# CRIMAC-WP4-Machine-learning/CRIMAC-classifiers-unet

Hardware: AMD Instinct MI355X
Metric: echogram patches/sec (4ch 256x256), training step (fwd+weighted CE+bwd+SGD) (higher is better)
Workload: dtype bf16; 1 GPU; BASELINE configs[1]: U-Net (depth 5, 64 filters) train step, batch 32 x 4x256x256 per GPU; global_batch=32, precision=bf16, start_filts=64, parallelism=dp1, ranks=1, launcher=single process

## Files before the change

### crimac_classifiers_unet_amd/csrc/elementwise.hip

```cpp
#include <stdarg.h>
#include <stdlib.h>

#include <mutex>

#include "common.h"

static thread_local char g_err[512] = "";
void crimac_set_error(const char* fmt, ...) {
  va_list ap;
  va_start(ap, fmt);
  vsnprintf(g_err, sizeof(g_err), fmt, ap);
  va_end(ap);
}
extern "C" const char* crimac_last_error(void) { return g_err; }
extern "C" int crimac_version(void) { return CRIMAC_ABI_VERSION; }
extern "C" int crimac_layer_desc_size(void) { return (int)sizeof(crimac_layer_desc); }

namespace {

#ifdef CRIMAC_STREAM_FORWARD
#define CRIMAC_ROW(x, M) (x)
#else
#define CRIMAC_ROW(x, M) ((M) - 1 - (x))
#endif
// ... 606 lines not shown
      for (int j = 0; j < 8; ++j) {
        int best = 0;
        float bv = av[0][j];
#pragma unroll
        for (int d = 1; d < 4; ++d)
          if (av[d][j] > bv) { bv = av[d][j]; best = d; }
        arg[j] = best;
      }
#pragma unroll
      for (int d = 0; d < 4; ++d) {
        float o[8];
        if (ds) load8s(ds + pix[d] * ds_ld + c0, o);
#pragma unroll
        for (int j = 0; j < 8; ++j) {
          o[j] = (ds ? o[j] : 0.f) + (arg[j] == d ? g[j] : 0.f);
          if constexpr (BNB) o[j] = storage_round<T>(o[j]);
        }
        if (da) store8(da + pix[d] * da_ld + c0, o);
        if constexpr (BNB) bnb_accum_v(k, yv[d], o, d1, d2);
      }
    }
  }
  if constexpr (BNB) bnb_flush(bnb, lds, C, c0, d1, d2, 256);
}

__device__ __forceinline__ float bn_bwd_dy(float yv, float g, float sc, float sh, float mu, float is, float k1, float k2) {
#pragma clang fp contract(off)
  const float act = __builtin_fmaf(yv, sc, sh);
  const float dz = act > 0.f ? g : 0.f;
  const float xh = (yv - mu) * is;
  return sc * __builtin_fmaf(-xh, k2, dz - k1);
}

template <typename T>
__global__ __launch_bounds__(256) void bn_bwd_reduce_kernel(const T* __restrict__ da, long da_ld,
                                                            const T* __restrict__ y, long y_ld,
                                                            const float* __restrict__ scale,
                                                            const float* __restrict__ shift,
                                                            const float* __restrict__ mean,
                                                            const float* __restrict__ invstd, long M,
                                                            int C, double* sum_dz, double* sum_dzx) {
  const int c0t = (threadIdx.x % (C / 8)) * 8;
  float sc[8], sh[8], mu[8], is[8];
#pragma unroll
  for (int j = 0; j < 8; ++j) {
    sc[j] = scale[c0t + j]; sh[j] = shift[c0t + j]; mu[j] = mean[c0t + j]; is[j] = invstd[c0t + j];
  }
  colreduce<T, double, 2>(M, C,
                          [&](long m, int c0, float (&q0)[8], float (&q1)[8]) {
                            float g[8], yv[8];
                            load8(da + m * da_ld + c0, g);
                            load8(y + m * y_ld + c0, yv);
#pragma unroll
                            for (int j = 0; j < 8; ++j) {
                              const float act = yv[j] * sc[j] + sh[j];
                              const float dz = act > 0.f ? g[j] : 0.f;
                              q0[j] = dz;
                              q1[j] = dz * (yv[j] - mu[j]) * is[j];
                            }
                          },
                          sum_dz, sum_dzx);
}

template <typename T, typename TD = T>
__global__ __launch_bounds__(256) void bn_bwd_apply_kernel(
    const T* __restrict__ da, long da_ld, const T* __restrict__ y, long y_ld,
// ... 141 lines not shown
    load8s(dp + r * dp_ld + c0, g);
    long pix[4];
#pragma unroll
    for (int d = 0; d < 4; ++d) {
      pix[d] = (b * H + 2 * yp + (d >> 1)) * (long)W + 2 * xp + (d & 1);
      load8s(y + pix[d] * y_ld + c0, yv[d]);
#pragma unroll
      for (int j = 0; j < 8; ++j) av[d][j] = storage_round<TA>(fmaxf(yv[d][j] * sc[j] + sh[j], 0.f));
    }
    int arg[8];
#pragma unroll
    for (int j = 0; j < 8; ++j) {
      int best = 0;
      float bv = av[0][j];
#pragma unroll
      for (int d = 1; d < 4; ++d)
        if (av[d][j] > bv) { bv = av[d][j]; best = d; }
      arg[j] = best;
    }
#pragma unroll
    for (int d = 0; d < 4; ++d) {
      float o[8];
      if (ds) load8s(ds + pix[d] * ds_ld + c0, o);
#pragma unroll
      for (int j = 0; j < 8; ++j) {
        const float dav = storage_round<T>((ds ? o[j] : 0.f) + (arg[j] == d ? g[j] : 0.f));
        o[j] = bn_bwd_dy(yv[d][j], dav, sc[j], sh[j], mu[j], is[j], k1[j], k2[j]);
      }
      store8(dy + pix[d] * dy_ld + c0, o);
    }
  }
}

template <typename T, int NC, typename TR = T>
__global__ __launch_bounds__(256) void head_fwd_kernel(const T* __restrict__ x, long x_ld, int Cin,
                                                       const float* __restrict__ w,
                                                       const float* __restrict__ bias,
                                                       float* __restrict__ logits, long npix, long HW,
                                                       int softmax, const float* __restrict__ bn_scale,
                                                       const float* __restrict__ bn_shift) {
  const int lp = Cin / 8;
  const int sub = threadIdx.x % lp;
  float bsc[8], bsh[8];
#pragma unroll
  for (int j = 0; j < 8; ++j) {
    bsc[j] = bn_scale ? bn_scale[sub * 8 + j] : 1.f;
    bsh[j] = bn_scale ? bn_shift[sub * 8 + j] : 0.f;
  }
  float wr[NC][8];
#pragma unroll
  for (int o = 0; o < NC; ++o)
#pragma unroll
    for (int j = 0; j < 8; ++j) wr[o][j] = w[o * Cin + sub * 8 + j];
  const long ppb = 256 / lp;
  for (long p0 = (long)blockIdx.x * ppb; p0 < npix; p0 += (long)gridDim.x * ppb) {
    const long p = p0 + threadIdx.x / lp;
    float acc[NC];
#pragma unroll
    for (int o = 0; o < NC; ++o) acc[o] = 0.f;
    if (p < npix) {
      float v[8];
      load8(x + p * x_ld + sub * 8, v);
      if (bn_scale) {
#pragma unroll
        for (int j = 0; j < 8; ++j) v[j] = storage_round<TR>(fmaxf(v[j] * bsc[j] + bsh[j], 0.f));
      }
// ... 150 lines not shown
  long pb[UNR], phw[UNR];
#pragma unroll
  for (int u = 0; u < UNR; ++u) { pb[u] = (p + u * step) / HW; phw[u] = (p + u * step) % HW; }
  for (; p < npix; p += UNR * step) {
    float g[UNR][NC], v[UNR][8], yv[UNR][8];
    bool ok[UNR];
#pragma unroll
    for (int u = 0; u < UNR; ++u) {
      const long pu = p + u * step;
      ok[u] = pu < npix;
      if (phw[u] >= HW) { phw[u] -= HW; pb[u] += 1; }
      if (ok[u]) {
#pragma unroll
        for (int o = 0; o < NC; ++o) g[u][o] = dl[(pb[u] * NC + o) * HW + phw[u]];
        if (x) load8s(x + pu * x_ld + sub * 8, v[u]);
        if constexpr (BNB) load8s(reinterpret_cast<const T*>(bnb.y) + pu * bnb.y_ld + sub * 8, yv[u]);
      }
      pb[u] += step_b;
      phw[u] += step_hw;
    }
#pragma unroll
    for (int u = 0; u < UNR; ++u) {
      if (!ok[u]) continue;
      const long pu = p + u * step;
      float o8[8];
      if constexpr (BNB) {
        if (!x) {
#pragma unroll
          for (int j = 0; j < 8; ++j) v[u][j] = storage_round<TX>(fmaxf(yv[u][j] * k.sc[j] + k.sh[j], 0.f));
        }
      }
#pragma unroll
      for (int j = 0; j < 8; ++j) {
        float s = 0.f;
#pragma unroll
        for (int o = 0; o < NC; ++o) { s += g[u][o] * wr[o][j]; gw[o][j] += g[u][o] * v[u][j]; }
        o8[j] = s;
      }
      if (sub == 0)
#pragma unroll
        for (int o = 0; o < NC; ++o) gb[o] += g[u][o];
      if constexpr (BNB) {
#pragma unroll
        for (int j = 0; j < 8; ++j) o8[j] = storage_round<T>(o8[j]);
      }
      store8(dx + pu * dx_ld + sub * 8, o8);
      if constexpr (BNB) bnb_accum_v(k, yv[u], o8, d1, d2);
    }
  }
#pragma unroll
  for (int o = 0; o < NC; ++o) {
#pragma unroll
    for (int j = 0; j < 8; ++j) atomicAdd(&lds[o * Cin + sub * 8 + j], gw[o][j]);
    if (sub == 0) atomicAdd(&lds[NC * Cin + o], gb[o]);
  }
  __syncthreads();
  for (int i = threadIdx.x; i < NC * Cin; i += 256) atomicAdd(&dw[i], lds[i]);
  if (threadIdx.x < NC) atomicAdd(&db[threadIdx.x], lds[NC * Cin + threadIdx.x]);
  if constexpr (BNB) bnb_flush(bnb, lds_bnb, Cin, sub * 8, d1, d2, 256);
}

__device__ __forceinline__ long load_label(const void* labels, int nbytes, long i) {
  if (nbytes == 8) return ((const long long*)labels)[i];
  if (nbytes == 4) return ((const int*)labels)[i];
  return ((const short*)labels)[i];
}

template <int NC>
__global__ __launch_bounds__(256) void wce_fwd_kernel(const float* __restrict__ logits,
                                                      const void* __restrict__ labels, int lbytes,
                                                      const float* __restrict__ cw, int ignore,
                                                      long npix, long HW, double* sums) {
  __shared__ double red[2][4];
  double s0 = 0.0, s1 = 0.0;
  auto pixel = [&](long y, const float (&z)[NC]) {
    if (y == ignore) return;
    float mx = -INFINITY;
#pragma unroll
    for (int o = 0; o < NC; ++o) mx = fmaxf(mx, z[o]);
// ... 531 lines not shown
    return head_fwd_launch<hp_t, hp_t>(x, x_ld, Cin, w, b, logits, B * HW, HW, ncls, softmax, bn_scale, bn_shift, ST);
  }
  CRIMAC_FOR_STORAGE(prec, T, return head_fwd_launch<T>(x, x_ld, Cin, w, b, logits, B * HW, HW, ncls, softmax, bn_scale,
                                                        bn_shift, ST));
}

template <typename T, typename TX = T>
static int head_bwd_launch(const float* dl, const void* x, long x_ld, int Cin, const float* w, void* dx,
                           long dx_ld, float* dw, float* db, long npix, long HW, int ncls, const BnbArgs& bnb,
                           hipStream_t st) {
  const int lp = Cin / 8;
  int grid = grid_for(npix, (256 / lp) * 32);
  if (grid > 1024) grid = 1024;
  const size_t lds = (size_t)(ncls * Cin + ncls + (bnb.sum_dz ? 2 * Cin : 0)) * sizeof(float);
#define HB(NC, BNB)                                                                                          \
  hipLaunchKernelGGL((head_bwd_kernel<T, NC, BNB, TX>), dim3(whole_rounds(head_bwd_kernel<T, NC, BNB, TX>, lds, grid)), dim3(256), lds, st, dl, (const TX*)x, x_ld,   \
                     Cin, w, (T*)dx, dx_ld, dw, db, npix, HW, bnb)
  if (bnb.sum_dz) {
    if (ncls == 2) HB(2, true); else if (ncls == 3) HB(3, true); else HB(4, true);
  } else {
    if (ncls == 2) HB(2, false); else if (ncls == 3) HB(3, false); else HB(4, false);
  }
#undef HB
  CRIMAC_LAUNCH_CHECK();
  return CRIMAC_OK;
}

extern "C" int crimac_head_bwd(int prec, const float* dlogits, const void* x, long x_ld, int Cin,
                               const float* w, void* dx, long dx_ld, float* dw, float* db, int B, int H,
                               int W, int ncls, const void* bnb_y, long bnb_y_ld, const float* bnb_vec,
                               long bnb_stride, double* stat_sum, double* stat_sumsq, int stat_replicas,
                               void* stream) {
  PREC_OK("head_bwd");
  CRIMAC_REQUIRE(dlogits && w && dx && dw && db && B > 0 && H > 0 && W > 0, "head_bwd: bad arguments");
  CRIMAC_REQUIRE(x || (bnb_y && stat_sum), "head_bwd: x may only be NULL together with the fused BatchNorm sums");
  CRIMAC_REQUIRE(ncls >= 2 && ncls <= 4, "head_bwd: ncls=%d unsupported (2..4)", ncls);
  CRIMAC_REQUIRE(head_cin_ok(Cin) && (!x || (x_ld >= Cin && x_ld % 8 == 0)) && dx_ld >= Cin && dx_ld % 8 == 0,
                 "head_bwd: Cin=%d must be 8*2^k <= 512", Cin);
  CRIMAC_REQUIRE(bnb_args_ok(bnb_y, bnb_y_ld, bnb_vec, bnb_stride, stat_sum, stat_sumsq, stat_replicas, Cin),
                 "head_bwd: bad arguments of the fused BatchNorm-backward sums");
  const long HW = (long)H * W;
  const BnbArgs bnb{bnb_y, bnb_y_ld, bnb_vec, bnb_stride, stat_sum, stat_sumsq, stat_replicas};
  CRIMAC_FOR_STORAGE2(prec, T, TX, return (head_bwd_launch<T, TX>(dlogits, x, x_ld, Cin, w, dx, dx_ld, dw, db, B * HW, HW, ncls,
                                                                    bnb, ST)));
}

extern "C" int crimac_wce_fwd(const float* logits, const void* labels, int label_bytes,
                              const float* class_w, int ncls, int ignore_index, int B, int H, int W,
                              double* sums, void* stream) {
  CRIMAC_REQUIRE(logits && labels && class_w && sums && B > 0 && H > 0 && W > 0, "wce_fwd: bad arguments");
  CRIMAC_REQUIRE(label_bytes == 2 || label_bytes == 4 || label_bytes == 8, "wce_fwd: label_bytes=%d", label_bytes);
  CRIMAC_REQUIRE(ncls >= 2 && ncls <= 4, "wce_fwd: ncls=%d unsupported (2..4)", ncls);
  const long HW = (long)H * W, npix = B * HW;
  int grid = grid_for(npix, 256 * 8);
  if (grid > 512) grid = 512;
#define WF(NC)                                                                                     \
  hipLaunchKernelGGL(wce_fwd_kernel<NC>, dim3(grid), dim3(256), 0, ST, logits, labels, label_bytes, \
                     class_w, ignore_index, npix, HW, sums)
  if (ncls == 2) WF(2); else if (ncls == 3) WF(3); else WF(4);
#undef WF
  CRIMAC_LAUNCH_CHECK();
  return CRIMAC_OK;
}

extern "C" int crimac_wce_bwd(const float* logits, const void* labels, int label_bytes,
                              const float* class_w, int ncls, int ignore_index, int B, int H, int W,
                              const double* sums, float upstream, float* dlogits, void* stream) {
  CRIMAC_REQUIRE(logits && labels && class_w && sums && dlogits && B > 0 && H > 0 && W > 0,
                 "wce_bwd: bad arguments");
  CRIMAC_REQUIRE(label_bytes == 2 || label_bytes == 4 || label_bytes == 8, "wce_bwd: label_bytes=%d", label_bytes);
  CRIMAC_REQUIRE(ncls >= 2 && ncls <= 4, "wce_bwd: ncls=%d unsupported (2..4)", ncls);
  const long HW = (long)H * W, npix = B * HW;
  const int grid = grid_for(npix, 256 * 4);
#define WB(NC)                                                                                     \
  hipLaunchKernelGGL(wce_bwd_kernel<NC>, dim3(whole_rounds(wce_bwd_kernel<NC>, 0, grid)), dim3(256), 0, ST, logits, labels, label_bytes, \
                     class_w, ignore_index, npix, HW, sums, upstream, dlogits)
  if (ncls == 2) WB(2); else if (ncls == 3) WB(3); else WB(4);
// ... 51 lines not shown
```

### crimac_classifiers_unet_amd/engine.py

```python
from __future__ import annotations

import ctypes as C
import os

import torch

from . import hip
from .hip import Act, call, ptr


def _on_device(fn):
    import functools

    @functools.wraps(fn)
    def wrapped(self, *a, **kw):
        if getattr(self, "device", None) is None:
            self.bind()
        dev = self.device
        if dev is None or dev.type != "cuda":
            return fn(self, *a, **kw)
        with torch.cuda.device(dev):
            return fn(self, *a, **kw)
    return wrapped

# ... 605 lines not shown
        if t is None or tuple(t.shape) != tuple(shape) or t.dtype != dtype:
            t = torch.empty(shape, dtype=dtype, device=self.device)
            self._bufs[key] = t
        return t

    def _wfrag_geometry(self, B, H, W):
        es = 4 if self.is_hp else 2
        small = (B * H * W - 1) * (2 * self.sf) * es + 2 * self.sf * es < (1 << 31)
        if small == getattr(self, "_wfrag_on", True):
            return
        self._wfrag_on = small
        for pks in (self.pk_main, self.pk_eval, self.pk16):
            for key, pk in pks.items():
                ok = pk.get("frag_ok") or (self.pk_main.get(key, {}).get("frag_ok", (False, False)) if pks is self.pk_eval else None)
                if ok is None:
                    continue
                if "fwd_frag" in pk:
                    pk["fwd_frag"] = bool(small and ok[0])
                if "dg_frag" in pk:
                    pk["dg_frag"] = bool(small and ok[1])
        self._ltab = self._ltab16 = None
        self._packed_groups = set()
        self._train_pack_dirty = self._eval_pack_dirty = True

    def _geom(self, B, H, W):
        self._wfrag_geometry(B, H, W)
        D = self.depth
        if H % (2 ** (D - 1)) or W % (2 ** (D - 1)):
            raise ValueError(f"H, W must be divisible by {2 ** (D - 1)} (got {H}x{W})")
        return [(H >> i, W >> i, B * (H >> i) * (W >> i)) for i in range(D)]

    fuse_bn_bwd = True
    fuse_unpool_apply = None
    fuse_head_bn = True

    def _conv3x3(self, x: Act, pk, bias, out: Act, B, H, W, cin, cout, relu, dgrad=False, cin_real=None,
                 stats=None, bnb=None, cols=None, out_planes=False, stat_reps=None):
        flops = 2.0 * 9 * (cin_real or cin) * cout * B * H * W
        relu = (hip.EPI_RELU if relu else 0) | (hip.EPI_OUT_PLANES if (out_planes and self.is_hp) else 0)
        if pk.get("narrow"):
            return self._conv3x3_narrow(x, pk, bias, out, B, H, W, cin, cout, relu, dgrad, stats, cols, stat_reps, flops)
        if self.is_hp and cin_real is not None and cin_real <= 4 and cin == CIN_PAD and not dgrad:
            relu |= hip.EPI_CIN4
        w_hi, w_lo = ptr(pk["dg_hi" if dgrad else "fwd_hi"]), ptr(pk["dg_lo" if dgrad else "fwd_lo"])
        if pk.get("dg_frag" if dgrad else "fwd_frag"):
            relu |= hip.EPI_WFRAG
        prec = self.prec_bwd if dgrad else self.prec
        mode, s0, s1, by, by_ld, bvec = 0, None, None, None, 0, None
        reps = stat_reps or self._nrep(cout)
        if stats is not None:
            mode, s0, s1 = 1, ptr(stats[0]), ptr(stats[1])
        elif bnb is not None and self.fuse_bn_bwd:
            blk, y = bnb
            mode, s0, s1 = 2, ptr(self._stat(blk, 0)), ptr(self._stat(blk, 1))
            by, by_ld, bvec = y.p, y.ld, ptr(self._bnf(blk, 0))
        if cols is not None:
            call("crimac_conv3x3_cols", prec, x.p, x.ld, B, H, W, cin, cout, w_hi, w_lo, ptr(bias),
                 out.p, out.ld, relu, mode, s0, s1, reps, by, by_ld, bvec, self.cmax,
                 cols[0], cols[1], flops=flops * cols[1] / cout, mfmas=hip.MFMAS_PER_PRODUCT[prec])
            return mode != 0
        call("crimac_conv3x3", prec, x.p, x.ld, B, H, W, cin, cout, w_hi, w_lo, ptr(bias),
             out.p, out.ld, relu, mode, s0, s1, reps, by, by_ld, bvec, self.cmax,
             flops=flops, mfmas=hip.MFMAS_PER_PRODUCT[prec])
        return mode != 0

    def _conv3x3_narrow(self, x: Act, pk, bias, out: Act, B, H, W, cin, cout, flags, dgrad, stats, cols, stat_reps, flops):
# ... 317 lines not shown
                    self._bn_act(b2, y2, a2, None, B, h, w, M)
                saved[f"d{j}"] = (cur, catA, y1, a1, y2, a2)
            else:
                pe1, pe2 = self.pk_eval[b1.conv_key], self.pk_eval[b2.conv_key]
                self._conv3x3(catA, pe1, pe1["bias"], a1, B, h, w, 2 * c, c, relu=True, out_planes=True)
                self._conv3x3(a1, pe2, pe2["bias"], a2, B, h, w, c, c, relu=True, out_planes=True)
            cur = a2
        logits = out if out is not None else torch.empty((B, self.n_classes, H, W), dtype=torch.float32,
                                                         device=self.device)
        if self.lmi:
            if meta is None:
                raise ValueError("UNet_LateMetInject needs the metadata tensor")
            w64, wm = self._lmi_weights()
            call("crimac_head_fwd", self.prec, cur.p, cur.ld, self.sf, ptr(w64), ptr(self.P["conv_final.bias"]),
                 ptr(logits), B, H, W, self.n_classes, 0,
                 ptr(self._bnf(head_bn, 2)) if head_bn is not None else None,
                 ptr(self._bnf(head_bn, 3)) if head_bn is not None else None)
            m = self._buf("lmi.m", (B * H * W,), torch.float32)
            call("crimac_meta_mlp_fwd", ptr(meta), self.meta_channels, B, H, W, *self._mlp(), ptr(m))
            call("crimac_meta_inject_fwd", ptr(m), ptr(wm), ptr(logits), B, H, W, self.n_classes, 1 if softmax else 0)
            saved["meta"] = meta
        else:
            call("crimac_head_fwd", self.prec, cur.p, cur.ld, self.sf, ptr(self.P["conv_final.weight"]),
                 ptr(self.P["conv_final.bias"]), ptr(logits), B, H, W, self.n_classes, 1 if softmax else 0,
                 ptr(self._bnf(head_bn, 2)) if head_bn is not None else None,
                 ptr(self._bnf(head_bn, 3)) if head_bn is not None else None)
        saved["head_in"] = cur if head_bn is None else None
        self.saved = saved if training else None
        if training:
            self.forward_generation += 1
        return logits

    def _block_bwd(self, tag, b, da: Act, y: Act, x_in: Act, B, h, w, M, dx_out: Act, reduce_done=False,
                   next_bn=None, bias_from_stats=None, unpool_src=None):
        world = self._sync_world()
        folded = reduce_done and self.fold_bn_finalize and world == 1
        if folded:
            pass
        elif reduce_done:
            call("crimac_sum_replicas", ptr(self._stat(b, 0)), self._nrep(b.cout), b.cout, b.cout,
                 ptr(self._stat(b, 2)), None, ptr(self._stat(b, 1)), ptr(self._stat(b, 3)))
        else:
            call("crimac_bn_bwd_reduce", self.prec, da.p, da.ld, y.p, y.ld, ptr(self._bnf(b, 2)),
                 ptr(self._bnf(b, 3)), ptr(self._bnf(b, 0)), ptr(self._bnf(b, 1)), M, b.cout,
                 ptr(self._stat(b, 2)), ptr(self._stat(b, 3)))
        dy = Act(self._buf(f"{tag}.dy", (M, b.cout), torch.float16 if self.bwd16 else None), b.cout)
        prec_apply = self.prec_bwd if self.bwd16 else self.prec
        dgamma, dbeta = self.G[b.bn_key + ".weight"], self.G[b.bn_key + ".bias"]
        if world > 1:
            import torch.distributed as dist
            dgamma.copy_(self._stat(b, 3))
            dbeta.copy_(self._stat(b, 2))
            dist.all_reduce(self._stat_pair(b), group=UNetEngine._bn_group)
            scr = self._buf("g.syncbn.scratch", (2, self.cmax), torch.float32)
            dgamma, dbeta = scr[0], scr[1]
        if unpool_src is not None:
            if not folded:
                raise RuntimeError("unpool_src needs the folded BatchNorm-backward path")
            dp_, ds_ = unpool_src
            call("crimac_unpool_bn_bwd_apply_replicas", prec_apply, dp_.p, dp_.ld, ds_.p if ds_ is not None else None,
                 ds_.ld if ds_ is not None else 0, y.p, y.ld, ptr(self._bnf(b, 0)), self.cmax, ptr(self._stat(b, 0)),
                 ptr(self._stat(b, 1)), self._nrep(b.cout), M, dy.p, dy.ld, B, h, w, b.cout, ptr(dgamma), ptr(dbeta))
        elif folded:
            call("crimac_bn_bwd_apply_replicas", prec_apply, da.p, da.ld, y.p, y.ld, ptr(self._bnf(b, 0)), self.cmax,
                 ptr(self._stat(b, 0)), ptr(self._stat(b, 1)), self._nrep(b.cout), M, M, b.cout, dy.p, dy.ld,
                 ptr(dgamma), ptr(dbeta))
        else:
            call("crimac_bn_bwd_apply", prec_apply, da.p, da.ld, y.p, y.ld, ptr(self._bnf(b, 2)),
                 ptr(self._bnf(b, 3)), ptr(self._bnf(b, 0)), ptr(self._bnf(b, 1)), ptr(self._stat(b, 2)),
                 ptr(self._stat(b, 3)), M, M * world, b.cout, dy.p, dy.ld, ptr(dgamma), ptr(dbeta), None)
        self._wgrad(self.prec_bwd, 0, dy.p, dy.ld, b.cout, x_in.p, x_in.ld, b.cin_pad, B, h, w, b.conv_key,
                    flops=2.0 * 9 * b.cin * b.cout * B * h * w)
        fused = False
        if dx_out is not None:
            stats = None
            if bias_from_stats is not None:
                per = 2 * STAT_REPLICAS * 2 * self.cmax
                lvl = bias_from_stats[2]
                scr = self.bias_scr[lvl * per:(lvl + 1) * per]
                stats = (scr[:per // 2], scr[per // 2:])
            C_up = bias_from_stats[1] if bias_from_stats is not None else 0
            side = self._side[0] if (self._side is not None and len(self._side) == 1) else None
            side_ok = side is not None and not self._gloo_ranks()
            if b.narrow and bias_from_stats is not None:
                self._conv3x3(dy, self.pk[b.conv_key], None, dx_out, B, h, w, b.cout, b.cin, relu=False, dgrad=True,
                              stats=stats, cols=(0, C_up), out_planes=True)
                if side_ok:
                    ev = self._side_events[self._side_i % len(self._side_events)]
                    self._side_i += 1
                    ev.record()
                    with torch.cuda.stream(side):
                        side.wait_event(ev)
                        self._conv3x3(dy, self.pk[b.conv_key], None, dx_out, B, h, w, b.cout, b.cin, relu=False,
                                      dgrad=True, cols=(C_up, C_up))
                        done = torch.cuda.Event()
# ... 85 lines not shown
        if [g for g, _ in bounds] != sorted(starts) or bounds[-1][1] != 0 or not bounds[0][1] < lo_dec:
            raise RuntimeError("unexpected parameter order in the flat buffer")
        for k, (o, _, _) in self.layout.items():
            if (o >= lo_dec) != (k.startswith(dec) or k.startswith("conv_final") or k.startswith("post_processing_weights")):
                raise RuntimeError(f"unexpected parameter order in the flat buffer at {k}")
        ranges, hi = [(lo_dec, self.n_flat)], lo_dec
        for _, lo in bounds:
            ranges.append((lo, hi))
            hi = lo
        return ranges

    @_on_device
    def backward(self, dlogits, on_ready=None, before_join=None):
        ranges = self.grad_ranges() if on_ready is not None else None
        s = self.saved
        if s is None:
            raise RuntimeError("backward() needs a preceding train-mode forward()")
        B, H, W = s["B"], s["H"], s["W"]
        geo = self._geom(B, H, W)
        D = self.depth
        self._skip_done = {}
        self._unpacked = {}
        self._wg_pending, self._wg_launches = [], 0
        self._dup16 = {}
        self._plan_dw(B, H, W)
        self.flat_g.zero_()
        if not self.use_wgrad_partials:
            self.dw_packed.zero_()
        self.stat[2:].zero_()
        self.bias_scr.zero_()
        dlogits = dlogits.contiguous().float()
        head_in = s["head_in"]
        h, w, M = geo[0]
        d_cur = Act(self._buf("g.head", (M, self.sf)), self.sf)
        head_fused = self.fuse_bn_bwd and D >= 2
        if head_in is None and not head_fused:
            raise RuntimeError("head input was not materialised (fuse_head_bn) but the fused BatchNorm sums are off")
        w_head, g_head = ptr(self.P["conv_final.weight"]), self.G["conv_final.weight"]
        if self.lmi:
            w64, wm = self._lmi_weights()
            g64 = self._buf("lmi.g64", (self.n_classes, self.sf), torch.float32)
            gwm = self._buf("lmi.gwm", (self.n_classes,), torch.float32)
            g64.zero_()
            gwm.zero_()
            pre = "post_processing_weights.main."
            call("crimac_meta_bwd", ptr(dlogits), ptr(s["meta"]), self.meta_channels, B, H, W, self.n_classes, ptr(wm),
                 *self._mlp(), ptr(gwm), *[ptr(self.G[pre + k]) for k in
                                          ("0.weight", "0.bias", "2.weight", "2.bias", "4.weight", "4.bias")])
            w_head, g_head = ptr(w64), g64
        call("crimac_head_bwd", self.prec, ptr(dlogits), head_in.p if head_in is not None else None,
             head_in.ld if head_in is not None else 0, self.sf,
             w_head, d_cur.p, d_cur.ld, ptr(g_head),
             ptr(self.G["conv_final.bias"]), B, H, W, self.n_classes,
             *self._bnb_args(self.dec[D - 2][1], s[f"d{D - 2}"][4] if head_fused else None))
        if self.lmi:
            gw = self.G["conv_final.weight"].view(self.n_classes, self.sf + 1)
            gw[:, :self.sf].copy_(g64)
            gw[:, self.sf].copy_(gwm)
        skip_grad = {}
        cur_done = head_fused
        for j in reversed(range(D - 1)):
            L = D - 2 - j
            h, w, M = geo[L]
            c = self.sf * 2 ** L
            u = self.ups[j]
            b1, b2 = self.dec[j]
            x_prev, catA, y1, a1, y2, a2 = s[f"d{j}"]
            da1 = Act(self._buf(f"g.d{j}.a1", (M, c)), c)
            fused = self._block_bwd(f"g.d{j}.2", b2, d_cur, y2, a1, B, h, w, M, da1, next_bn=(b1, y1),
                                    reduce_done=cur_done)
            dcat = Act(self._buf(f"g.d{j}.cat", (M, 2 * c)), 2 * c)
            self._block_bwd(f"g.d{j}.1", b1, da1, y1, catA, B, h, w, M, dcat, reduce_done=fused,
                            bias_from_stats=(self.G[u.key + ".bias"], c, j))
            dup = self._dup16.get(j) or dcat.slice(0, c)
            skip_grad[L] = dcat.slice(c, c)
            hp, wp, Mp = geo[L + 1]
            if u.up1x1:
                dup = self._up1x1_adjoint(dup, u, B, hp, wp)
                self._wgrad1x1(dup, x_prev, u, Mp)
            else:
                self._wgrad(self.prec_bwd, 1, x_prev.p, x_prev.ld, u.cin, dup.p, dup.ld, u.cout, B, hp, wp, u.key,
                            flops=2.0 * 4 * u.cin * u.cout * B * hp * wp)
            d_prev = Act(self._buf(f"g.d{j}.xprev", (Mp, u.cin)), u.cin)
            nxt = (self.dec[j - 1][1], s[f"d{j - 1}"][4]) if j > 0 else (self.enc[D - 1][1], s[f"e{D - 1}"][3])
            cur_done = self._upconv_dgrad(dup, u, d_prev, B, hp, wp, next_bn=nxt)
            d_cur = d_prev
        self._unpack_group(0, on_ready, ranges[0] if ranges else None)
        d_pool = None
        for i in reversed(range(D)):
            h, w, M = geo[i]
            c = self.sf * 2 ** i
            b1, b2 = self.enc[i]
            x_in, y1, a1, y2, a2 = s[f"e{i}"]
            unpool_src = None
            if i == D - 1:
                da2 = d_cur
            else:
                ds = skip_grad[i]
                ev = self._skip_done.pop(D - 2 - i, None)
                if ev is not None:
                    torch.cuda.current_stream().wait_event(ev)
                if (self.fuse_unpool_apply and self.fuse_bn_bwd and self.fold_bn_finalize
                        and self._sync_world() == 1):
# ... 256 lines not shown
```

### crimac_classifiers_unet_amd/hip.py

```python
from __future__ import annotations

import ctypes as C
import os

import torch

from . import build as _build

PREC_BF16 = 0
PREC_F32X3 = 1
PREC_F32X6 = 2
PREC_FP16 = 3
PREC_F32H3 = 4
PREC_H3P = 5
PREC_H3F_BWD = 6
PREC_NAMES = {"bf16": PREC_BF16, "f32x3": PREC_F32X3, "f32x6": PREC_F32X6, "fp16": PREC_FP16, "f32h3": PREC_F32H3,
              "h3p": PREC_H3P, "h3f": PREC_H3P}
MFMAS_PER_PRODUCT = {PREC_BF16: 1, PREC_FP16: 1, PREC_F32X3: 3, PREC_F32H3: 3, PREC_H3P: 3, PREC_F32X6: 6, PREC_H3F_BWD: 1}
PREC_PLANES = {PREC_BF16: 1, PREC_F32X3: 2, PREC_F32X6: 3, PREC_FP16: 1, PREC_F32H3: 2, PREC_H3P: 2}
PLANES_FP16 = 1 | 16 | 32
PLANES_F32H3 = 2 | 16 | (8 << 8)
PLANES_FWD_FRAG = 65536
PLANES_INTERLEAVED = 64
PLANES_H3P = 2 | 16 | 32 | PLANES_INTERLEAVED | 128 | (8 << 8)
PREC_PLANES_ARG = {PREC_BF16: 1, PREC_F32X3: 2, PREC_F32X6: 3, PREC_FP16: PLANES_FP16, PREC_F32H3: PLANES_F32H3,
                   PREC_H3P: PLANES_H3P}
EPI_RELU, EPI_OUT_PLANES, EPI_CIN4 = 1, 2, 4
EPI_WFRAG = 16
EPI_WROWS = 32
NARROW_DGRAD = 64
LAYER_FWD_FRAG, LAYER_DG_FRAG = 16, 32
LAYER_CONV3X3, LAYER_UPCONV2X2, LAYER_CONV1X1 = 0, 1, 2
PREC_BACKWARD = {PREC_F32H3: PREC_F32X3}
PREC_16BIT = (PREC_BF16, PREC_FP16)

ABI_VERSION = 10

_vp, _i, _l, _f = C.c_void_p, C.c_int, C.c_long, C.c_float

SIGNATURES = {
    "crimac_igemm_conv": [_i, _vp, _l, _i, _i, _i, _i, _i, _i, _i, _i, _i, _i, _i, _vp, _vp, _vp, _i,
                          _vp, _l, _i, _i, _i, _vp],
    "crimac_conv3x3": [_i, _vp, _l, _i, _i, _i, _i, _i, _vp, _vp, _vp, _vp, _l, _i, _i, _vp, _vp, _i,
                       _vp, _l, _vp, _l, _vp],
    "crimac_conv3x3_pool": [_i, _vp, _l, _i, _i, _i, _i, _i, _vp, _vp, _vp, _vp, _l, _i, _vp, _l, _vp],
    "crimac_conv3x3_cols": [_i, _vp, _l, _i, _i, _i, _i, _i, _vp, _vp, _vp, _vp, _l, _i, _i, _vp, _vp, _i,
                            _vp, _l, _vp, _l, _i, _i, _vp],
    "crimac_upconv2x2_dgrad_bnb": [_vp, _l, _i, _i, _i, _i, _i, _vp, _vp, _l, _vp, _l, _vp, _l, _vp, _vp, _i, _vp],
    "crimac_upconv2x2_dgrad_bnb_prec": [_i, _vp, _l, _i, _i, _i, _i, _i, _vp, _vp, _l, _vp, _l, _vp, _l, _vp, _vp, _i,
                                        _vp],
    "crimac_sum_replicas": [_vp, _i, _l, _i, _vp, _vp, _vp, _vp, _vp],
    "crimac_wgrad": [_i, _i, _vp, _l, _i, _vp, _l, _i, _i, _i, _i, _vp, _i, _vp],
    "crimac_wgrad_partials": [_i, _i, _vp, _l, _i, _vp, _l, _i, _i, _i, _i, _vp, _l, _i, _vp],
    "crimac_wgrad_group": [_i, _vp, _i, _i, _vp, _i, _vp, _vp, _vp],
    "crimac_conv1x1_up2x": [_i, _vp, _l, _i, _i, _i, _i, _i, _vp, _vp, _vp, _vp, _vp, _l, _vp],
    "crimac_up2x_adjoint": [_i, _vp, _l, _i, _i, _i, _i, _vp, _l, _vp],
    "crimac_conv1x1_dgrad": [_i, _vp, _l, _i, _i, _i, _i, _i, _vp, _vp, _vp, _l, _vp],
    "crimac_conv1x1_wgrad": [_i, _vp, _l, _i, _vp, _l, _i, _l, _vp, _vp],
    "crimac_conv3x3_narrow": [_i, _vp, _l, _i, _i, _i, _i, _i, _vp, _i, _i, _i, _vp, _vp, _vp, _l, _vp, _vp, _i, _i,
                              _vp],
    "crimac_upconv2x2_narrow": [_i, _vp, _l, _i, _i, _i, _i, _i, _vp, _vp, _vp, _l, _i, _vp],
    "crimac_upconv2x2_dgrad_narrow": [_i, _vp, _l, _i, _i, _i, _i, _i, _vp, _vp, _l, _vp],
    "crimac_pack_conv3x3": [_vp, _i, _i, _i, _vp, _i, _vp, _vp, _vp, _vp, _vp],
    "crimac_pack_upconv2x2": [_vp, _i, _i, _i, _vp, _vp, _vp, _vp, _vp],
    "crimac_unpack_wgrad_conv3x3": [_vp, _i, _i, _i, _vp, _vp],
    "crimac_unpack_wgrad_upconv2x2": [_vp, _i, _i, _vp, _vp],
    "crimac_pack_layers": [_vp, _i, _i, _vp],
    "crimac_unpack_wgrad_layers": [_vp, _i, _vp],
    "crimac_nchw_to_nhwc": [_i, _vp, _vp, _i, _i, _i, _i, _l, _vp],
    "crimac_colstats": [_i, _vp, _l, _l, _i, _vp, _vp, _vp],
    "crimac_colsum_f32": [_i, _vp, _l, _l, _i, _vp, _vp],
    "crimac_bn_finalize": [_vp, _vp, _i, _l, _i, _vp, _vp, _f, _f, _vp, _vp, _vp, _vp, _vp, _vp, _vp, _vp],
    "crimac_bn_act_pool": [_i, _vp, _l, _vp, _vp, _i, _vp, _l, _vp, _l, _i, _i, _i, _i, _vp],
    "crimac_bn_train_act_pool": [_i, _vp, _l, _vp, _vp, _i, _l, _vp, _vp, _f, _f, _vp, _vp, _vp, _vp, _l, _i, _vp, _l,
                                 _vp, _l, _i, _i, _i, _i, _vp],
    "crimac_unpool_add": [_i, _vp, _l, _vp, _l, _vp, _l, _vp, _l, _i, _i, _i, _i, _vp, _l, _vp, _l, _vp, _vp, _i,
                          _vp],
    "crimac_bn_bwd_reduce": [_i, _vp, _l, _vp, _l, _vp, _vp, _vp, _vp, _l, _i, _vp, _vp, _vp],
    "crimac_bn_bwd_apply": [_i, _vp, _l, _vp, _l, _vp, _vp, _vp, _vp, _vp, _vp, _l, _l, _i, _vp, _l, _vp,
                            _vp, _vp, _vp],
    "crimac_bn_bwd_apply_replicas": [_i, _vp, _l, _vp, _l, _vp, _l, _vp, _vp, _i, _l, _l, _i, _vp, _l, _vp, _vp, _vp],
    "crimac_unpool_bn_bwd_apply_replicas": [_i, _vp, _l, _vp, _l, _vp, _l, _vp, _l, _vp, _vp, _i, _l, _vp, _l, _i, _i, _i, _i,
                                            _vp, _vp, _vp],
    "crimac_head_fwd": [_i, _vp, _l, _i, _vp, _vp, _vp, _i, _i, _i, _i, _i, _vp, _vp, _vp],
    "crimac_head_bwd": [_i, _vp, _vp, _l, _i, _vp, _vp, _l, _vp, _vp, _i, _i, _i, _i, _vp, _l, _vp, _l, _vp, _vp,
                        _i, _vp],
    "crimac_softmax_nchw": [_vp, _vp, _i, _i, _i, _i, _vp],
    "crimac_wce_fwd": [_vp, _vp, _i, _vp, _i, _i, _i, _i, _i, _vp, _vp],
    "crimac_wce_bwd": [_vp, _vp, _i, _vp, _i, _i, _i, _i, _i, _vp, _f, _vp, _vp],
    "crimac_sgd_momentum": [_vp, _vp, _vp, _l, _f, _f, _f, _i, _vp],
    "crimac_grad_overflow_flag": [_vp, _l, _vp, _vp],
    "crimac_sgd_momentum_guarded": [_vp, _vp, _vp, _l, _f, _f, _f, _i, _vp, _vp],
    "crimac_meta_planes": [_vp, _i, _i, _i, _i, C.c_double, _vp, _i, _vp, _i, _vp, _i, _vp, _vp],
    "crimac_meta_mlp_fwd": [_vp, _i, _i, _i, _i, _vp, _vp, _vp, _vp, _vp, _vp, _vp, _vp],
    "crimac_meta_inject_fwd": [_vp, _vp, _vp, _i, _i, _i, _i, _i, _vp],
    "crimac_meta_bwd": [_vp, _vp, _i, _i, _i, _i, _i, _vp, _vp, _vp, _vp, _vp, _vp, _vp, _vp, _vp, _vp, _vp, _vp, _vp,
                        _vp, _vp],
    "crimac_gather_patches": [_i, _vp, _i, _i, _i, _vp, _i, _i, _i, _vp, _l, _vp],
    "crimac_gather_patches_memm": [_i, _vp, _i, _i, _i, _vp, _i, _i, _i, _vp, _l, _vp, _vp],
    "crimac_gather_patches_memm_meta": [_i, _vp, _i, _i, _i, _vp, _i, _i, _i, _vp, _l, _vp, _i, _i, C.c_double, _vp, _i,
                                        _vp, _i, _vp, _i, _vp, _vp],
    "crimac_scatter_patches_ex": [_vp, _i, _vp, _i, _i, _i, _i, _i, _i, _i, _vp, _vp, _i, _i, _vp, _i, _i, _vp, _i, _i,
                                  _i, _i, _vp, _i, _vp],
    "crimac_gather_eval_crops": [_vp, _i, _i, _i, _vp, _vp, _i, _i, _i, _i, _vp, _vp, _vp],
    "crimac_augment_db_nhwc": [_i, _vp, _vp, _i, _vp, _vp, _vp, _i, _f, _f, _i, _i, _i, _i, _l, C.c_ulonglong,
                               _i, _i, _i, _vp],
    "crimac_augment_db_meta_nhwc": [_i, _vp, _vp, _i, _vp, _vp, _vp, _i, _f, _f, _i, _i, _i, _i, _l, C.c_ulonglong,
                                    _i, _i, _i, _i, _vp],
    "crimac_augment_flip_planes": [_vp, _vp, _i, _i, _i, _i, C.c_ulonglong, _i, _vp],
    "crimac_refine_labels": [_vp, _i, _vp, _vp, _i, _f, _f, _i, _vp, _i, _i, _i, _i, _vp],
    "crimac_pr_histogram": [_vp, _i, _vp, _i, _i, _i, _i, _vp, _vp, _vp],
    "crimac_mfma_calibrate": [_i, _i, _vp, _vp],
    "crimac_labels_test_transform": [_vp, _i, _vp, _i, _f, _f, _vp, _vp, _i, _i, _vp, _i, _i, _i, _i, _i, _i, _vp, _i, _i,
                                     _i, _i],
    "crimac_labels_extend_mask": [_vp, _vp, _i, _vp, _vp, _i, _i, _i, _i, _i],
    "crimac_scatter_patches": [_vp, _i, _vp, _i, _i, _i, _i, _i, _i, _i, _vp, _vp, _i, _i, _vp, _i, _i,
                               _i, _vp, _vp],
    "crimac_seabed_columns": [_vp, _i, _l, _i, _i, _i, _i, _vp, _vp, _l, _vp],
}
# ... 121 lines not shown
```

### include/crimac_unet_hip.h

```cpp
#ifndef CRIMAC_UNET_HIP_H_
#define CRIMAC_UNET_HIP_H_

#ifdef __cplusplus
extern "C" {
#endif

#define CRIMAC_OK 0
#define CRIMAC_ERR_INVALID (-22)
#define CRIMAC_ERR_LAUNCH (-5)

#define CRIMAC_PREC_BF16 0
#define CRIMAC_PREC_F32X3 1
#define CRIMAC_PREC_F32X6 2
#define CRIMAC_PREC_FP16 3
#define CRIMAC_PREC_F32H3 4
#define CRIMAC_PREC_H3P 5
#define CRIMAC_PREC_MAX 5
#define CRIMAC_PREC_H3F_BWD 6
#define CRIMAC_F32H3_WSHIFT 8
#define CRIMAC_PLANES_FWD_FP16 16
#define CRIMAC_PLANES_DG_FP16 32
#define CRIMAC_PLANES_FP16 (1 | CRIMAC_PLANES_FWD_FP16 | CRIMAC_PLANES_DG_FP16)
#define CRIMAC_PLANES_F32H3 (2 | CRIMAC_PLANES_FWD_FP16 | (CRIMAC_F32H3_WSHIFT << 8))
#define CRIMAC_PLANES_INTERLEAVED 64
#define CRIMAC_PLANES_FWD_FRAG 65536
#define CRIMAC_PLANES_DG_SCALED 128
#define CRIMAC_PLANES_H3P (2 | CRIMAC_PLANES_FWD_FP16 | CRIMAC_PLANES_DG_FP16 | CRIMAC_PLANES_INTERLEAVED | \
                           CRIMAC_PLANES_DG_SCALED | (CRIMAC_F32H3_WSHIFT << 8))

#define CRIMAC_EPI_RELU 1
#define CRIMAC_EPI_OUT_PLANES 2
#define CRIMAC_EPI_CIN4 4
#define CRIMAC_EPI_STAT_RAW 8
#define CRIMAC_EPI_WFRAG 16
#define CRIMAC_EPI_WROWS 32

#define CRIMAC_ABI_VERSION 10
int crimac_version(void);
int crimac_layer_desc_size(void);
const char* crimac_last_error(void);


int crimac_igemm_conv(int prec, const void* in, long in_ld, int B, int Hi, int Wi, int Ho, int Wo,
                      int Cin, int N, int ntaps, int tw, int pad, int stride, const void* w_hi,
                      const void* w_lo, const float* bias, int bias_mod, void* out, long out_ld,
                      int relu, int out_mode, int cout_up, void* stream);

int crimac_upconv2x2_dgrad_bnb(const void* dy, long dy_ld, int B, int H, int W, int Cout, int Cin,
                               const void* w_dg_hi, void* dx, long dx_ld, const void* bnb_y, long bnb_y_ld,
                               const float* bnb_vec, long bnb_stride, double* stat_sum, double* stat_sumsq,
                               int stat_replicas, void* stream);
int crimac_upconv2x2_dgrad_bnb_prec(int prec, const void* dy, long dy_ld, int B, int H, int W, int Cout, int Cin,
                                    const void* w_dg_hi, void* dx, long dx_ld, const void* bnb_y, long bnb_y_ld,
                                    const float* bnb_vec, long bnb_stride, double* stat_sum, double* stat_sumsq,
                                    int stat_replicas, void* stream);


int crimac_conv3x3(int prec, const void* in, long in_ld, int B, int H, int W, int Cin, int N,
                   const void* w_hi, const void* w_lo, const float* bias, void* out, long out_ld,
                   int relu, int stat_mode, double* stat_sum, double* stat_sumsq, int stat_replicas,
                   const void* bnb_y, long bnb_y_ld, const float* bnb_vec, long bnb_stride, void* stream);

int crimac_conv3x3_cols(int prec, const void* in, long in_ld, int B, int H, int W, int Cin, int N,
                   const void* w_hi, const void* w_lo, const float* bias, void* out, long out_ld,
                   int relu, int stat_mode, double* stat_sum, double* stat_sumsq, int stat_replicas,
                   const void* bnb_y, long bnb_y_ld, const float* bnb_vec, long bnb_stride, int n_first, int n_count, void* stream);

int crimac_conv3x3_pool(int prec, const void* in, long in_ld, int B, int H, int W, int Cin, int N,
                        const void* w_hi, const void* w_lo, const float* bias, void* out, long out_ld, int relu,
                        void* pool_out, long pool_ld, void* stream);
// ... 78 lines not shown
                             float momentum, float* running_mean, float* running_var,
                             long long* num_batches_tracked, float* bn_vec, long bn_stride, int relu, void* out,
                             long out_ld, void* pool_out, long pool_ld, int B, int H, int W, int C, void* stream);
int crimac_unpool_add(int prec, const void* dp, long dp_ld, const void* a, long a_ld, const void* ds,
                      long ds_ld, void* da, long da_ld, int B, int H, int W, int C, const void* bnb_y,
                      long bnb_y_ld, const float* bnb_vec, long bnb_stride, double* stat_sum,
                      double* stat_sumsq, int stat_replicas, void* stream);
int crimac_bn_bwd_reduce(int prec, const void* da, long da_ld, const void* y, long y_ld,
                         const float* scale, const float* shift, const float* mean,
                         const float* invstd, long M, int C, double* sum_dz, double* sum_dz_xhat,
                         void* stream);
int crimac_bn_bwd_apply(int prec, const void* da, long da_ld, const void* y, long y_ld,
                        const float* scale, const float* shift, const float* mean, const float* invstd,
                        const double* sum_dz, const double* sum_dz_xhat, long M, long count, int C, void* dy,
                        long dy_ld, float* dgamma, float* dbeta, float* dbias, void* stream);

int crimac_bn_bwd_apply_replicas(int prec, const void* da, long da_ld, const void* y, long y_ld, const float* bn_vec,
                                 long bn_stride, const double* sum_dz, const double* sum_dz_xhat, int replicas, long M,
                                 long count, int C, void* dy, long dy_ld, float* dgamma, float* dbeta, void* stream);

int crimac_unpool_bn_bwd_apply_replicas(int prec, const void* dp, long dp_ld, const void* ds, long ds_ld, const void* y,
                                        long y_ld, const float* bn_vec, long bn_stride, const double* sum_dz,
                                        const double* sum_dz_xhat, int replicas, long count, void* dy, long dy_ld, int B,
                                        int H, int W, int C, float* dgamma, float* dbeta, void* stream);


int crimac_head_fwd(int prec, const void* x, long x_ld, int Cin, const float* w, const float* b,
                    float* logits, int B, int H, int W, int ncls, int softmax, const float* bn_scale,
                    const float* bn_shift, void* stream);
int crimac_head_bwd(int prec, const float* dlogits, const void* x, long x_ld, int Cin, const float* w,
                    void* dx, long dx_ld, float* dw, float* db, int B, int H, int W, int ncls,
                    const void* bnb_y, long bnb_y_ld, const float* bnb_vec, long bnb_stride, double* stat_sum,
                    double* stat_sumsq, int stat_replicas, void* stream);
int crimac_softmax_nchw(const float* logits, float* out, int B, int ncls, int H, int W, void* stream);

int crimac_wce_fwd(const float* logits, const void* labels, int label_bytes, const float* class_w,
                   int ncls, int ignore_index, int B, int H, int W, double* sums, void* stream);
int crimac_wce_bwd(const float* logits, const void* labels, int label_bytes, const float* class_w,
                   int ncls, int ignore_index, int B, int H, int W, const double* sums,
                   float upstream, float* dlogits, void* stream);
int crimac_sgd_momentum(float* p, float* g, float* v, long n, float lr, float momentum,
                        float grad_scale, int zero_grad, void* stream);
int crimac_grad_overflow_flag(const float* g, long n, int* state, void* stream);
int crimac_sgd_momentum_guarded(float* p, float* g, float* v, long n, float lr, float momentum,
                                float grad_scale, int zero_grad, int* state, void* stream);



int crimac_gather_patches(int prec, const float* data, int C, int Wd, int H, const int* centres, int P,
                          int ph, int pw, void* out, long ld, void* stream);
int crimac_gather_patches_memm(int prec, const float* data, int C, int Wd, int H, const int* centres, int P, int ph,
                               int pw, void* out, long ld, const short* border_labels, void* stream);
int crimac_gather_patches_memm_meta(int prec, const float* data, int C, int Wd, int H, const int* centres, int P,
                                    int ph, int pw, void* out, long ld, const short* border_labels, int db_scaled,
                                    int flags, double portion_year, const double* portion_day, int n_day,
                                    const double* time_diff, int n_td, const long long* seabed, int n_sb,
                                    const int* meta_centres, void* stream);

int crimac_scatter_patches(const float* probs, int ncls, const int* centres, int P, int ph, int pw,
                           int overlap, int start_ping, int n_chunk, int H, const short* labels,
                           const unsigned char* seabed_mask, int mask_ping0, int mask_pings,
                           const float* data0, int data_ping0, int data_pings, int seabed_pad, float* out,
                           void* stream);
int crimac_scatter_patches_ex(const float* probs, int ncls, const int* centres, int P, int ph, int pw, int overlap,
                              int start_ping, int n_chunk, int H, const short* labels,
                              const unsigned char* seabed_mask, int mask_ping0, int mask_pings, const int* seabed,
// ... 75 lines not shown
```

Baseline: 2914 patches/s.

## Recompute head dgrad inside BN-backward apply to skip head gradient buffer

The head backward no longer writes its per-pixel input gradient (M x 64 channels) when the folded single-rank BatchNorm path is active. The following BN-backward apply kernel instead recomputes that gradient on the fly from the logits gradient and the head weights. This removes one full-resolution activation write and its later read. The cost is reading dlogits in NCHW layout with scattered per-pixel loads and a few extra FMAs per element. Both kernels now share a dot-product helper with FMA contraction disabled, so the two computations round identically.

```diff
diff --git a/crimac_classifiers_unet_amd/csrc/elementwise.hip b/crimac_classifiers_unet_amd/csrc/elementwise.hip
--- a/crimac_classifiers_unet_amd/csrc/elementwise.hip
+++ b/crimac_classifiers_unet_amd/csrc/elementwise.hip
@@ -662,6 +662,15 @@
   return sc * __builtin_fmaf(-xh, k2, dz - k1);
 }
 
+template <int NC>
+__device__ __forceinline__ float head_dx(const float (&g)[NC], const float (&wr)[NC][8], int j) {
+#pragma clang fp contract(off)
+  float s = 0.f;
+#pragma unroll
+  for (int o = 0; o < NC; ++o) s = __builtin_fmaf(g[o], wr[o][j], s);
+  return s;
+}
+
 template <typename T>
 __global__ __launch_bounds__(256) void bn_bwd_reduce_kernel(const T* __restrict__ da, long da_ld,
                                                             const T* __restrict__ y, long y_ld,
@@ -869,6 +878,71 @@
   }
 }
 
+template <typename T, typename TD, int NC>
+__global__ __launch_bounds__(256) __attribute__((amdgpu_waves_per_eu(CRIMAC_BNB_APPLY_WAVES)))
+void head_bn_bwd_apply_kernel(
+    const float* __restrict__ dl, const float* __restrict__ w, long HW, const T* __restrict__ y, long y_ld,
+    const float* __restrict__ scale, const float* __restrict__ shift, const float* __restrict__ mean,
+    const float* __restrict__ invstd, const double* __restrict__ sum_dz, const double* __restrict__ sum_dzx, long M,
+    long count, int C, TD* __restrict__ dy, long dy_ld, float* dgamma, float* dbeta, int nrep) {
+  extern __shared__ __attribute__((aligned(16))) unsigned char bn_smem[];
+  float* k12 = reinterpret_cast<float*>(bn_smem + 512 * sizeof(double));
+  const double invM = 1.0 / (double)count;
+  {
+    const bool writer = blockIdx.x == 0;
+    replica_sums_block(sum_dz, sum_dzx, nrep, C, reinterpret_cast<double*>(bn_smem), [&](int c, double s1, double s2) {
+      k12[c] = (float)(s1 * invM);
+      k12[C + c] = (float)(s2 * invM);
+      if (writer) { dbeta[c] = (float)s1; dgamma[c] = (float)s2; }
+    });
+    __syncthreads();
+  }
+  const int cpr = C / 8;
+  const int rpi = 256 / cpr > 0 ? 256 / cpr : 1;
+  const int chunk = threadIdx.x % cpr, rl = threadIdx.x / cpr;
+  if (rl >= rpi) return;
+  const int c0 = chunk * 8;
+  float sc[8], sh[8], mu[8], is[8], k1[8], k2[8], wr[NC][8];
+#pragma unroll
+  for (int j = 0; j < 8; ++j) {
+    sc[j] = scale[c0 + j]; sh[j] = shift[c0 + j]; mu[j] = mean[c0 + j]; is[j] = invstd[c0 + j];
+    k1[j] = k12[c0 + j];
+    k2[j] = k12[C + c0 + j];
+#pragma unroll
+    for (int o = 0; o < NC; ++o) wr[o][j] = w[o * C + c0 + j];
+  }
+  const long stride = (long)gridDim.x * rpi;
+#ifdef CRIMAC_BNB_APPLY_U
+  constexpr int U = CRIMAC_BNB_APPLY_U;
+#else
+  constexpr int U = CRIMAC_BNB_APPLY_WAVES >= 4 ? 2 : 4;
+#endif
+  for (long m = (long)blockIdx.x * rpi + rl; m < M; m += U * stride) {
+    float g[U][NC], yv[U][8];
+#pragma unroll
+    for (int u = 0; u < U; ++u)
+      if (m + u * stride < M) {
+        const long row = CRIMAC_ROW(m + u * stride, M);
+        long b, hw;
+        pix_split(row, HW, b, hw);
+#pragma unroll
+        for (int o = 0; o < NC; ++o) g[u][o] = dl[(b * NC + o) * HW + hw];
+        load8s(y + row * y_ld + c0, yv[u]);
+      }
+#pragma unroll
+    for (int u = 0; u < U; ++u) {
+      if (m + u * stride >= M) continue;
+      float o[8];
+#pragma unroll
+      for (int j = 0; j < 8; ++j) {
+        const float dav = storage_round<T>(head_dx<NC>(g[u], wr, j));
+        o[j] = bn_bwd_dy(yv[u][j], dav, sc[j], sh[j], mu[j], is[j], k1[j], k2[j]);
+      }
+      store8(dy + CRIMAC_ROW(m + u * stride, M) * dy_ld + c0, o);
+    }
+  }
+}
+
 template <typename T, int NC, typename TR = T>
 __global__ __launch_bounds__(256) void head_fwd_kernel(const T* __restrict__ x, long x_ld, int Cin,
                                                        const float* __restrict__ w,
@@ -1085,10 +1159,9 @@
       }
 #pragma unroll
       for (int j = 0; j < 8; ++j) {
-        float s = 0.f;
-#pragma unroll
-        for (int o = 0; o < NC; ++o) { s += g[u][o] * wr[o][j]; gw[o][j] += g[u][o] * v[u][j]; }
-        o8[j] = s;
+#pragma unroll
+        for (int o = 0; o < NC; ++o) gw[o][j] += g[u][o] * v[u][j];
+        o8[j] = head_dx<NC>(g[u], wr, j);
       }
       if (sub == 0)
 #pragma unroll
@@ -1097,7 +1170,7 @@
 #pragma unroll
         for (int j = 0; j < 8; ++j) o8[j] = storage_round<T>(o8[j]);
       }
-      store8(dx + pu * dx_ld + sub * 8, o8);
+      if (dx) store8(dx + pu * dx_ld + sub * 8, o8);
       if constexpr (BNB) bnb_accum_v(k, yv[u], o8, d1, d2);
     }
   }
@@ -1695,10 +1768,11 @@
                                long bnb_stride, double* stat_sum, double* stat_sumsq, int stat_replicas,
                                void* stream) {
   PREC_OK("head_bwd");
-  CRIMAC_REQUIRE(dlogits && w && dx && dw && db && B > 0 && H > 0 && W > 0, "head_bwd: bad arguments");
+  CRIMAC_REQUIRE(dlogits && w && dw && db && B > 0 && H > 0 && W > 0, "head_bwd: bad arguments");
   CRIMAC_REQUIRE(x || (bnb_y && stat_sum), "head_bwd: x may only be NULL together with the fused BatchNorm sums");
+  CRIMAC_REQUIRE(dx || (bnb_y && stat_sum), "head_bwd: dx may only be NULL together with the fused BatchNorm sums");
   CRIMAC_REQUIRE(ncls >= 2 && ncls <= 4, "head_bwd: ncls=%d unsupported (2..4)", ncls);
-  CRIMAC_REQUIRE(head_cin_ok(Cin) && (!x || (x_ld >= Cin && x_ld % 8 == 0)) && dx_ld >= Cin && dx_ld % 8 == 0,
+  CRIMAC_REQUIRE(head_cin_ok(Cin) && (!x || (x_ld >= Cin && x_ld % 8 == 0)) && (!dx || (dx_ld >= Cin && dx_ld % 8 == 0)),
                  "head_bwd: Cin=%d must be 8*2^k <= 512", Cin);
   CRIMAC_REQUIRE(bnb_args_ok(bnb_y, bnb_y_ld, bnb_vec, bnb_stride, stat_sum, stat_sumsq, stat_replicas, Cin),
                  "head_bwd: bad arguments of the fused BatchNorm-backward sums");
@@ -1706,6 +1780,33 @@
   const BnbArgs bnb{bnb_y, bnb_y_ld, bnb_vec, bnb_stride, stat_sum, stat_sumsq, stat_replicas};
   CRIMAC_FOR_STORAGE2(prec, T, TX, return (head_bwd_launch<T, TX>(dlogits, x, x_ld, Cin, w, dx, dx_ld, dw, db, B * HW, HW, ncls,
                                                                     bnb, ST)));
+}
+
+extern "C" int crimac_head_bn_bwd_apply_replicas(int prec, const float* dlogits, const float* w, int ncls, const void* y,
+                                                 long y_ld, const float* bn_vec, long bn_stride, const double* sum_dz,
+                                                 const double* sum_dz_xhat, int replicas, long count, void* dy,
+                                                 long dy_ld, int B, int H, int W, int C, float* dgamma, float* dbeta,
+                                                 void* stream) {
+  PREC_OK_BWD16("head_bn_bwd_apply_replicas");
+  CRIMAC_REQUIRE(dlogits && w && y && bn_vec && bn_stride >= C && sum_dz && sum_dz_xhat && replicas >= 1 && dy && dgamma &&
+                     dbeta && B > 0 && H > 0 && W > 0,
+                 "head_bn_bwd_apply_replicas: bad arguments");
+  CRIMAC_REQUIRE(ncls >= 2 && ncls <= 4, "head_bn_bwd_apply_replicas: ncls=%d unsupported (2..4)", ncls);
+  CRIMAC_REQUIRE(head_cin_ok(C), "head_bn_bwd_apply_replicas: C=%d must be 8*2^k <= 512", C);
+  const long HW = (long)H * W, M = B * HW;
+  CRIMAC_REQUIRE(count == 0 || count >= M, "head_bn_bwd_apply_replicas: count smaller than the pixels of this call");
+  if (count == 0) count = M;
+  CRIMAC_REQUIRE(y_ld >= C && dy_ld >= C && y_ld % 8 == 0 && dy_ld % 8 == 0, "head_bn_bwd_apply_replicas: bad pixel strides");
+  const int grid = colreduce_grid(M, C);
+  const size_t lds = 512 * sizeof(double) + 2 * (size_t)C * sizeof(float);
+#define HBA(T, TD, NC)                                                                                                  \
+  hipLaunchKernelGGL((head_bn_bwd_apply_kernel<T, TD, NC>), dim3(whole_rounds(head_bn_bwd_apply_kernel<T, TD, NC>, lds, grid)), dim3(256), lds, ST, dlogits, w, HW,      \
+                     (const T*)y, y_ld, bn_vec + 2 * bn_stride, bn_vec + 3 * bn_stride, bn_vec, bn_vec + bn_stride, sum_dz,    \
+                     sum_dz_xhat, M, count, C, (TD*)dy, dy_ld, dgamma, dbeta, replicas)
+  CRIMAC_FOR_STORAGE2(prec, T, TD, { if (ncls == 2) HBA(T, TD, 2); else if (ncls == 3) HBA(T, TD, 3); else HBA(T, TD, 4); });
+#undef HBA
+  CRIMAC_LAUNCH_CHECK();
+  return CRIMAC_OK;
 }
 
 extern "C" int crimac_wce_fwd(const float* logits, const void* labels, int label_bytes,
diff --git a/crimac_classifiers_unet_amd/engine.py b/crimac_classifiers_unet_amd/engine.py
--- a/crimac_classifiers_unet_amd/engine.py
+++ b/crimac_classifiers_unet_amd/engine.py
@@ -661,6 +661,7 @@
 
     fuse_bn_bwd = True
     fuse_unpool_apply = None
+    fuse_head_apply = True
     fuse_head_bn = True
 
     def _conv3x3(self, x: Act, pk, bias, out: Act, B, H, W, cin, cout, relu, dgrad=False, cin_real=None,
@@ -1044,7 +1045,7 @@
         return logits
 
     def _block_bwd(self, tag, b, da: Act, y: Act, x_in: Act, B, h, w, M, dx_out: Act, reduce_done=False,
-                   next_bn=None, bias_from_stats=None, unpool_src=None):
+                   next_bn=None, bias_from_stats=None, unpool_src=None, head_src=None):
         world = self._sync_world()
         folded = reduce_done and self.fold_bn_finalize and world == 1
         if folded:
@@ -1073,6 +1074,13 @@
             call("crimac_unpool_bn_bwd_apply_replicas", prec_apply, dp_.p, dp_.ld, ds_.p if ds_ is not None else None,
                  ds_.ld if ds_ is not None else 0, y.p, y.ld, ptr(self._bnf(b, 0)), self.cmax, ptr(self._stat(b, 0)),
                  ptr(self._stat(b, 1)), self._nrep(b.cout), M, dy.p, dy.ld, B, h, w, b.cout, ptr(dgamma), ptr(dbeta))
+        elif head_src is not None:
+            if not folded:
+                raise RuntimeError("head_src needs the folded BatchNorm-backward path")
+            dl_, wh_ = head_src
+            call("crimac_head_bn_bwd_apply_replicas", prec_apply, ptr(dl_), wh_, self.n_classes, y.p, y.ld,
+                 ptr(self._bnf(b, 0)), self.cmax, ptr(self._stat(b, 0)), ptr(self._stat(b, 1)), self._nrep(b.cout), M,
+                 dy.p, dy.ld, B, h, w, b.cout, ptr(dgamma), ptr(dbeta))
         elif folded:
             call("crimac_bn_bwd_apply_replicas", prec_apply, da.p, da.ld, y.p, y.ld, ptr(self._bnf(b, 0)), self.cmax,
                  ptr(self._stat(b, 0)), ptr(self._stat(b, 1)), self._nrep(b.cout), M, M, b.cout, dy.p, dy.ld,
@@ -1224,8 +1232,9 @@
         dlogits = dlogits.contiguous().float()
         head_in = s["head_in"]
         h, w, M = geo[0]
-        d_cur = Act(self._buf("g.head", (M, self.sf)), self.sf)
         head_fused = self.fuse_bn_bwd and D >= 2
+        head_apply = self.fuse_head_apply and head_fused and self.fold_bn_finalize and self._sync_world() == 1
+        d_cur = None if head_apply else Act(self._buf("g.head", (M, self.sf)), self.sf)
         if head_in is None and not head_fused:
             raise RuntimeError("head input was not materialised (fuse_head_bn) but the fused BatchNorm sums are off")
         w_head, g_head = ptr(self.P["conv_final.weight"]), self.G["conv_final.weight"]
@@ -1242,7 +1251,7 @@
             w_head, g_head = ptr(w64), g64
         call("crimac_head_bwd", self.prec, ptr(dlogits), head_in.p if head_in is not None else None,
              head_in.ld if head_in is not None else 0, self.sf,
-             w_head, d_cur.p, d_cur.ld, ptr(g_head),
+             w_head, d_cur.p if d_cur is not None else None, d_cur.ld if d_cur is not None else 0, ptr(g_head),
              ptr(self.G["conv_final.bias"]), B, H, W, self.n_classes,
              *self._bnb_args(self.dec[D - 2][1], s[f"d{D - 2}"][4] if head_fused else None))
         if self.lmi:
@@ -1260,7 +1269,8 @@
             x_prev, catA, y1, a1, y2, a2 = s[f"d{j}"]
             da1 = Act(self._buf(f"g.d{j}.a1", (M, c)), c)
             fused = self._block_bwd(f"g.d{j}.2", b2, d_cur, y2, a1, B, h, w, M, da1, next_bn=(b1, y1),
-                                    reduce_done=cur_done)
+                                    reduce_done=cur_done,
+                                    head_src=(dlogits, w_head) if (head_apply and j == D - 2) else None)
             dcat = Act(self._buf(f"g.d{j}.cat", (M, 2 * c)), 2 * c)
             self._block_bwd(f"g.d{j}.1", b1, da1, y1, catA, B, h, w, M, dcat, reduce_done=fused,
                             bias_from_stats=(self.G[u.key + ".bias"], c, j))
diff --git a/crimac_classifiers_unet_amd/hip.py b/crimac_classifiers_unet_amd/hip.py
--- a/crimac_classifiers_unet_amd/hip.py
+++ b/crimac_classifiers_unet_amd/hip.py
@@ -34,7 +34,7 @@
 PREC_BACKWARD = {PREC_F32H3: PREC_F32X3}
 PREC_16BIT = (PREC_BF16, PREC_FP16)
 
-ABI_VERSION = 10
+ABI_VERSION = 11
 
 _vp, _i, _l, _f = C.c_void_p, C.c_int, C.c_long, C.c_float
 
@@ -85,6 +85,8 @@
     "crimac_head_fwd": [_i, _vp, _l, _i, _vp, _vp, _vp, _i, _i, _i, _i, _i, _vp, _vp, _vp],
     "crimac_head_bwd": [_i, _vp, _vp, _l, _i, _vp, _vp, _l, _vp, _vp, _i, _i, _i, _i, _vp, _l, _vp, _l, _vp, _vp,
                         _i, _vp],
+    "crimac_head_bn_bwd_apply_replicas": [_i, _vp, _vp, _i, _vp, _l, _vp, _l, _vp, _vp, _i, _l, _vp, _l, _i, _i, _i, _i,
+                                          _vp, _vp, _vp],
     "crimac_softmax_nchw": [_vp, _vp, _i, _i, _i, _i, _vp],
     "crimac_wce_fwd": [_vp, _vp, _i, _vp, _i, _i, _i, _i, _i, _vp, _vp],
     "crimac_wce_bwd": [_vp, _vp, _i, _vp, _i, _i, _i, _i, _i, _vp, _f, _vp, _vp],
diff --git a/include/crimac_unet_hip.h b/include/crimac_unet_hip.h
--- a/include/crimac_unet_hip.h
+++ b/include/crimac_unet_hip.h
@@ -35,7 +35,7 @@
 #define CRIMAC_EPI_WFRAG 16
 #define CRIMAC_EPI_WROWS 32
 
-#define CRIMAC_ABI_VERSION 10
+#define CRIMAC_ABI_VERSION 11
 int crimac_version(void);
 int crimac_layer_desc_size(void);
 const char* crimac_last_error(void);
@@ -180,6 +180,10 @@
                     void* dx, long dx_ld, float* dw, float* db, int B, int H, int W, int ncls,
                     const void* bnb_y, long bnb_y_ld, const float* bnb_vec, long bnb_stride, double* stat_sum,
                     double* stat_sumsq, int stat_replicas, void* stream);
+int crimac_head_bn_bwd_apply_replicas(int prec, const float* dlogits, const float* w, int ncls, const void* y, long y_ld,
+                                      const float* bn_vec, long bn_stride, const double* sum_dz,
+                                      const double* sum_dz_xhat, int replicas, long count, void* dy, long dy_ld, int B,
+                                      int H, int W, int C, float* dgamma, float* dbeta, void* stream);
 int crimac_softmax_nchw(const float* logits, float* out, int B, int ncls, int H, int W, void* stream);
 
 int crimac_wce_fwd(const float* logits, const void* labels, int label_bytes, const float* class_w,
```

Result: no change. 2918 patches/s, median of 6 (+0.1%).
